# JingwenWang95/DSP-SLAM

Hardware: AMD Instinct MI355X
Metric: objects/sec (2000 pts, 64-D code, 10 GN iters) (higher is better)
Workload: dtype f32 + f16 classifier

## Files before the change

dsp_slam_amd/csrc/mlp_kernel.hip:

```cpp
#include "dsp_internal.h"
#include "mlp_common.h"

namespace dsp {

#define FOR16(M) M(0) M(1) M(2) M(3) M(4) M(5) M(6) M(7) M(8) M(9) M(10) M(11) M(12) M(13) M(14) M(15)

template <int MODE>
__global__ __launch_bounds__(256, 1) void mlp_kernel(const MlpArgs a) {
    constexpr bool BWD = MODE >= 2;
    constexpr bool MASKS = MODE != 0;
    constexpr bool DOFWD = MODE != 3;
    extern __shared__ __attribute__((aligned(16))) char smem[];
    const int tid = threadIdx.x;
    const int lane = tid & 63;
    const int wave = __builtin_amdgcn_readfirstlane(tid >> 6);
    const int g = lane >> 4;
    const int pl = lane & 15;

    const DecoderLds lds = carve_lds(smem);
    float* const bias_l = lds.bias;
    float* const cb_l = lds.cb;
    unsigned short* const mask_l = lds.mask;
    char* ring_ptr = smem + LDS_HEAD_BYTES + (MASKS ? MASK_BYTES : 0);
    const unsigned ring0 = lds_addr(ring_ptr);

    const int n_tiles = *a.n_tiles;
    const int tile0 = a.tile_begin ? *a.tile_begin : 0;
    if (tile0 + (int)blockIdx.x >= n_tiles) return;
    if (a.clk && blockIdx.x == 0 && tid == 0) { a.clk[0] = clock64(); a.clk[1] = wall_clock64(); }
    stage_bias_table(a, bias_l, tid);

    int issue_pos = 0, issue_slot = 0, rd_slot = 0;
    const char* wbase = reinterpret_cast<const char*>(a.wstream) + wave * 4096;
    const unsigned lane_off = lane * 16;
    const int total_chunks = a.total_chunks;
    const char* isrc = wbase;
    unsigned idst = ring0 + wave * 4096;
    auto issue_next = [&]() {
        issue_pos = (issue_pos + 1 == total_chunks) ? 0 : issue_pos + 1;
        issue_slot = (issue_slot + 1 == NBUF) ? 0 : issue_slot + 1;
        isrc = wbase + (size_t)issue_pos * CHUNK_BYTES;
        idst = ring0 + issue_slot * CHUNK_BYTES + wave * 4096;
    };
    auto issue = [&]() {
        glds_quarter(isrc, lane_off, idst);
        issue_next();
    };
#pragma unroll
    for (int i = 0; i < NBUF - 1; ++i) issue();
    asm volatile("s_waitcnt vmcnt(%0)\n\ts_barrier" ::"n"(GLDS_PER_CHUNK * (NBUF - 2)) : "memory");
    f32x4 abuf[2 * PAIR_READS];
    static_assert(PAIR_READS == 2, "the prologue below reads the first group");
    abuf[0] = *reinterpret_cast<const f32x4*>(ring_ptr + lane * 16);
    abuf[1] = *reinterpret_cast<const f32x4*>(ring_ptr + lane * 16 + 1024);

    float sin_[128];
    f32x4 acc[32];
#pragma unroll
    for (int i = 0; i < 128; ++i) sin_[i] = 0.f;
#pragma unroll
    for (int i = 0; i < 32; ++i) acc[i] = (f32x4){0.f, 0.f, 0.f, 0.f};

    for (int tile = tile0 + blockIdx.x; tile < n_tiles; tile += gridDim.x) {
        const int4 td = a.tiles[tile];
        const int local = wave * WAVE_PTS + pl;
        const bool valid = local < td.y;
        const int pidx = td.x + (valid ? local : 0);
        const int src = (MODE <= 1 && a.index) ? a.index[pidx] : pidx;
        float4 pt = a.pts[src];
        float old_lp = 1.0f, guard_tol = 0.f;
        if (MODE <= 1 && a.guard) {
            if (valid && g == 0) old_lp = a.out_sdf[a.index ? src : pidx + td.w];
            guard_tol = 0.5f * __uint_as_float(a.guard[(size_t)td.z * a.guard_stride]);
        }
        if (!valid) pt = make_float4(0.f, 0.f, 0.f, 0.f);
        if (DOFWD) {
            stage_code_bias(a, cb_l, td.z, tid);
            __syncthreads();
#pragma unroll
            for (int o = 0; o < 8; ++o) {
                float pre[16];
#pragma unroll
                for (int j = 0; j < 4; ++j) {
                    const f32x4 p4 = layer0_rows(a, bias_l, cb_l, g, 16 * (4 * o + j), pt);
#pragma unroll
                    for (int r = 0; r < 4; ++r) pre[4 * j + r] = p4[r];
                }
                if (MASKS) {
                    unsigned bits = 0;
#pragma unroll
                    for (int k = 15; k >= 0; --k) push_mask_bit(bits, pre[k]);
                    mask_l[(0 * 8 + o) * 256 + tid] = (unsigned short)bits;
                }
#pragma unroll
                for (int k = 0; k < 16; ++k) sin_[16 * o + k] = relu1(pre[k]);
            }
        }
        float skipc[16];
        float skipx[3];
        float y = 0.f;
        float gfirst = 0.f;
#pragma unroll
        for (int i = 0; i < 16; ++i) skipc[i] = 0.f;
        skipx[0] = skipx[1] = skipx[2] = 0.f;

        auto seed_backward = [&](int slot) {
            const float d = 1.f - y * y;
#pragma unroll
            for (int o = 0; o < 8; ++o) {
                const unsigned bits = mask_l[(slot * 8 + o) * 256 + tid];
#pragma unroll
                for (int j = 0; j < 4; ++j) {
                    const f32x4 s4 = backward_seed_rows(a, bias_l, g, 4 * o + j, bits >> (4 * j), d);
#pragma unroll
                    for (int r = 0; r < 4; ++r) sin_[16 * o + 4 * j + r] = s4[r];
                }
            }
        };
        if (MODE == 3) {
            const int sidx = __float_as_int(pt.w);
            import_masks<8>(mask_words(a, sidx, g), valid, mask_l, tid);
            y = valid ? a.sdf_in[sidx] : 0.f;
            seed_backward(a.seed_slot);
        }

        for (int ps = 0; ps < a.n_pass; ++ps) {
            const PassDesc pd = a.pass[ps];
            if (pd.kind == 2) reinject_xyz(sin_, g, a.lat_tile, pt);
            else if (BWD && pd.kind == 5) gfirst = first_layer_xyz_grad(a, bias_l, g, sin_);

#pragma unroll
            for (int og = 0; og < 8; ++og) {
                if (og < pd.nog) {
                    f32x4 bias4[4];
                    if (pd.bias_row != -1) {
                        const float* bp = pass_bias_vec(pd.bias_row, bias_l, cb_l) + 64 * og + 4 * g;
#pragma unroll
                        for (int j = 0; j < 4; ++j) bias4[j] = *reinterpret_cast<const f32x4*>(bp + 16 * j);
                    } else {
#pragma unroll
                        for (int j = 0; j < 4; ++j) bias4[j] = (f32x4){0.f, 0.f, 0.f, 0.f};
                    }
#pragma unroll
                    for (int c = 0; c < 8; ++c) {
                        if (c < pd.nchunks) {
                            const int nx_slot = (rd_slot + 1 == NBUF) ? 0 : rd_slot + 1;
                            const char* cb = ring_ptr + rd_slot * CHUNK_BYTES + lane * 16;
                            const char* nb = ring_ptr + nx_slot * CHUNK_BYTES + lane * 16;
#pragma unroll
                            for (int s = 0; s < KSTEPS_PER_CHUNK; ++s) {
                                if (s == KSTEPS_PER_CHUNK / 2) {
                                    asm volatile("s_waitcnt vmcnt(%0)\n\ts_barrier" ::"n"(GLDS_PER_CHUNK * (NBUF - 3)) : "memory");
                                }
                                constexpr int RG = PAIR_READS;
                                if ((s % RG) == 0) {
                                    __builtin_amdgcn_s_waitcnt(0xC07F);
                                    __builtin_amdgcn_sched_barrier(0);
#pragma unroll
                                    for (int q = 0; q < RG; ++q) {
                                        const int sp = s + RG + q;
                                        abuf[sp % (2 * RG)] = (sp < KSTEPS_PER_CHUNK)
                                                           ? *reinterpret_cast<const f32x4*>(cb + sp * 1024)
                                                           : *reinterpret_cast<const f32x4*>(nb + (sp - KSTEPS_PER_CHUNK) * 1024);
                                    }
                                }
                                const f32x4 av = abuf[s % (2 * PAIR_READS)];
                                const float b = sin_[16 * c + s];
                                acc[4 * og + 0] = MFMA16(av.x, b, (c == 0 && s == 0) ? bias4[0] : acc[4 * og + 0]);
                                if (s == KSTEPS_PER_CHUNK / 2 + 0) { glds_set_dst(idst); glds_piece_m0<0>(isrc, lane_off, idst); };
                                if (s == KSTEPS_PER_CHUNK / 2 + 1) glds_piece_m0<1>(isrc, lane_off, idst);
                                if (s == KSTEPS_PER_CHUNK / 2 + 2) glds_piece_m0<2>(isrc, lane_off, idst);
                                if (s == KSTEPS_PER_CHUNK / 2 + 3) { glds_piece_m0<3>(isrc, lane_off, idst); issue_next(); }
                                acc[4 * og + 1] = MFMA16(av.y, b, (c == 0 && s == 0) ? bias4[1] : acc[4 * og + 1]);
                                acc[4 * og + 2] = MFMA16(av.z, b, (c == 0 && s == 0) ? bias4[2] : acc[4 * og + 2]);
                                acc[4 * og + 3] = MFMA16(av.w, b, (c == 0 && s == 0) ? bias4[3] : acc[4 * og + 3]);
                                __builtin_amdgcn_sched_barrier(0);
                            }
                            rd_slot = nx_slot;
                        }
                    }
                }
            }

#pragma unroll
            for (int og = 0; og < 8; ++og) {
                if (og < pd.nog) {
                    float v[16];
#pragma unroll
                    for (int j = 0; j < 4; ++j) {
                        v[4 * j + 0] = acc[4 * og + j].x; v[4 * j + 1] = acc[4 * og + j].y;
                        v[4 * j + 2] = acc[4 * og + j].z; v[4 * j + 3] = acc[4 * og + j].w;
                    }
                    if (pd.relu) {
                        if (MASKS) {
                            unsigned bits = 0;
#pragma unroll
                            for (int k = 15; k >= 0; --k) push_mask_bit(bits, v[k]);
                            mask_l[(pd.mask_slot * 8 + og) * 256 + tid] = (unsigned short)bits;
                        }
#pragma unroll
                        for (int k = 0; k < 16; ++k) v[k] = relu1(v[k]);
                    } else if (BWD && pd.mask_slot >= 0) {
                        if (pd.kind == 4) capture_skip_rows(a.lat_tile, og, v, skipx, skipc);
                        const unsigned bits = mask_l[(pd.mask_slot * 8 + og) * 256 + tid];
#pragma unroll
                        for (int k = 0; k < 16; ++k) v[k] = ((bits >> k) & 1u) ? v[k] : 0.f;
                    }
#pragma unroll
                    for (int k = 0; k < 16; ++k) sin_[16 * og + k] = v[k];
                }
            }

            if (DOFWD && ps == a.n_fwd - 1) {
                y = final_layer_sdf(a, bias_l, g, sin_);
                if (!BWD) {
                    if (a.guard) prepass_guard_tol(a, td.z, valid && g == 0, old_lp, y, guard_tol);
                    if (valid && g == 0) a.out_sdf[a.index ? src : pidx + td.w] = y;
                    if (MODE == 1 && valid && y > -a.th && y < a.th) {
                        export_masks<8>(mask_words(a, src, g), mask_l, tid);
                    }
                } else {
                    seed_backward(pd.mask_slot);
                }
            }
        }

        if (BWD) {
            write_jgrad_row(a.out_grad + (size_t)(pidx + td.w) * GRAD_STRIDE, valid, g, pl, sin_, skipc, skipx[0], skipx[1], skipx[2], gfirst, y);
            if (MODE == 2 && a.sdf_scatter && tile >= *a.scatter_tile_begin) scatter_sdf(a, td.z, valid && g == 3, pt, y);
        }
        asm volatile("s_waitcnt vmcnt(0)" ::: "memory");
    }
    asm volatile("s_waitcnt vmcnt(0)" ::: "memory");
    if (a.clk && blockIdx.x == 0 && tid == 0) { a.clk[2] = clock64(); a.clk[3] = wall_clock64(); }
}

static void (*const MLP_KERNELS[4])(const MlpArgs) = {mlp_kernel<0>, mlp_kernel<1>, mlp_kernel<2>, mlp_kernel<3>};

size_t mlp_lds_bytes(int mode) { return LDS_HEAD_BYTES + (mode != 0 ? MASK_BYTES : 0) + NBUF * CHUNK_BYTES; }

hipError_t mlp_prepare_device() {
    for (int i = 0; i < 4; ++i) {
        const hipError_t e = hipFuncSetAttribute(reinterpret_cast<const void*>(MLP_KERNELS[i]), hipFuncAttributeMaxDynamicSharedMemorySize, (int)mlp_lds_bytes(i));
        if (e != hipSuccess) return e;
    }
    return hipSuccess;
}

hipError_t launch_mlp(int mode, const MlpArgs& args, int n_blocks, hipStream_t stream) {
    hipLaunchKernelGGL(MLP_KERNELS[mode], dim3(n_blocks), dim3(256), mlp_lds_bytes(mode), stream, args);
    return hipGetLastError();
}

}
```

Measured before the change: 120.3.

## Double-buffer MFMA accumulators and seed bias tiles inside the MFMA stream

Replaces the 32-register accumulator array with two ping-pong 4-tile accumulator sets plus a separate output array. The bias seeding of the next output group and the copy-out of the previous group are interleaved into the first chunk's MFMA steps. A zero vector in LDS replaces the branch for passes without bias. The aim is to hide the bias loads and the conditional accumulator initialisation behind MFMA latency, at the cost of an extra register copy per tile, extra LDS, and possible register pressure.

After: 121.8, median of 6. 1.3% higher.

```diff
diff --git a/dsp_slam_amd/csrc/mlp_kernel.hip b/dsp_slam_amd/csrc/mlp_kernel.hip
--- a/dsp_slam_amd/csrc/mlp_kernel.hip
+++ b/dsp_slam_amd/csrc/mlp_kernel.hip
@@ -2,6 +2,8 @@
 #include "mlp_common.h"
 
 namespace dsp {
+
+constexpr int ZERO_VEC_BYTES = WIDTH * 4;
 
 #define FOR16(M) M(0) M(1) M(2) M(3) M(4) M(5) M(6) M(7) M(8) M(9) M(10) M(11) M(12) M(13) M(14) M(15)
 
@@ -23,11 +25,13 @@
     unsigned short* const mask_l = lds.mask;
     char* ring_ptr = smem + LDS_HEAD_BYTES + (MASKS ? MASK_BYTES : 0);
     const unsigned ring0 = lds_addr(ring_ptr);
+    float* const zero_l = reinterpret_cast<float*>(ring_ptr + NBUF * CHUNK_BYTES);
 
     const int n_tiles = *a.n_tiles;
     const int tile0 = a.tile_begin ? *a.tile_begin : 0;
     if (tile0 + (int)blockIdx.x >= n_tiles) return;
     if (a.clk && blockIdx.x == 0 && tid == 0) { a.clk[0] = clock64(); a.clk[1] = wall_clock64(); }
+    if (tid < ZERO_VEC_BYTES / 16) reinterpret_cast<float4*>(zero_l)[tid] = make_float4(0.f, 0.f, 0.f, 0.f);
     stage_bias_table(a, bias_l, tid);
 
     int issue_pos = 0, issue_slot = 0, rd_slot = 0;
@@ -55,11 +59,14 @@
     abuf[1] = *reinterpret_cast<const f32x4*>(ring_ptr + lane * 16 + 1024);
 
     float sin_[128];
-    f32x4 acc[32];
+    f32x4 acc[2][4];
+    f32x4 outv[32];
 #pragma unroll
     for (int i = 0; i < 128; ++i) sin_[i] = 0.f;
 #pragma unroll
-    for (int i = 0; i < 32; ++i) acc[i] = (f32x4){0.f, 0.f, 0.f, 0.f};
+    for (int i = 0; i < 32; ++i) outv[i] = (f32x4){0.f, 0.f, 0.f, 0.f};
+#pragma unroll
+    for (int i = 0; i < 8; ++i) acc[i >> 2][i & 3] = (f32x4){0.f, 0.f, 0.f, 0.f};
 
     for (int tile = tile0 + blockIdx.x; tile < n_tiles; tile += gridDim.x) {
         const int4 td = a.tiles[tile];
@@ -129,18 +136,21 @@
             if (pd.kind == 2) reinject_xyz(sin_, g, a.lat_tile, pt);
             else if (BWD && pd.kind == 5) gfirst = first_layer_xyz_grad(a, bias_l, g, sin_);
 
+            auto pin_vgpr = [](f32x4& t) __attribute__((always_inline)) { asm volatile("" : "=v"(t) : "0"(t)); };
+            const float* const seed_src = (pd.bias_row == -1 ? zero_l : pass_bias_vec(pd.bias_row, bias_l, cb_l)) + 4 * g;
+            auto seed_tile = [&](int og, int j) __attribute__((always_inline)) {
+                acc[og & 1][j] = *reinterpret_cast<const f32x4*>(seed_src + 64 * og + 16 * j);
+            };
+            auto read_out = [&](int og, int j) __attribute__((always_inline)) {
+                f32x4 t = acc[og & 1][j];
+                pin_vgpr(t);
+                outv[4 * og + j] = t;
+            };
+#pragma unroll
+            for (int j = 0; j < 4; ++j) seed_tile(0, j);
 #pragma unroll
             for (int og = 0; og < 8; ++og) {
                 if (og < pd.nog) {
-                    f32x4 bias4[4];
-                    if (pd.bias_row != -1) {
-                        const float* bp = pass_bias_vec(pd.bias_row, bias_l, cb_l) + 64 * og + 4 * g;
-#pragma unroll
-                        for (int j = 0; j < 4; ++j) bias4[j] = *reinterpret_cast<const f32x4*>(bp + 16 * j);
-                    } else {
-#pragma unroll
-                        for (int j = 0; j < 4; ++j) bias4[j] = (f32x4){0.f, 0.f, 0.f, 0.f};
-                    }
 #pragma unroll
                     for (int c = 0; c < 8; ++c) {
                         if (c < pd.nchunks) {
@@ -166,14 +176,21 @@
                                 }
                                 const f32x4 av = abuf[s % (2 * PAIR_READS)];
                                 const float b = sin_[16 * c + s];
-                                acc[4 * og + 0] = MFMA16(av.x, b, (c == 0 && s == 0) ? bias4[0] : acc[4 * og + 0]);
+                                f32x4 (&ac)[4] = acc[og & 1];
+                                ac[0] = MFMA16(av.x, b, ac[0]);
                                 if (s == KSTEPS_PER_CHUNK / 2 + 0) { glds_set_dst(idst); glds_piece_m0<0>(isrc, lane_off, idst); };
                                 if (s == KSTEPS_PER_CHUNK / 2 + 1) glds_piece_m0<1>(isrc, lane_off, idst);
                                 if (s == KSTEPS_PER_CHUNK / 2 + 2) glds_piece_m0<2>(isrc, lane_off, idst);
                                 if (s == KSTEPS_PER_CHUNK / 2 + 3) { glds_piece_m0<3>(isrc, lane_off, idst); issue_next(); }
-                                acc[4 * og + 1] = MFMA16(av.y, b, (c == 0 && s == 0) ? bias4[1] : acc[4 * og + 1]);
-                                acc[4 * og + 2] = MFMA16(av.z, b, (c == 0 && s == 0) ? bias4[2] : acc[4 * og + 2]);
-                                acc[4 * og + 3] = MFMA16(av.w, b, (c == 0 && s == 0) ? bias4[3] : acc[4 * og + 3]);
+                                constexpr int SSTEP[4] = {2, 4, 6, 12};
+#pragma unroll
+                                for (int j = 0; j < 4; ++j) {
+                                    if (og > 0 && c == 0 && s == 2 * j + 1) read_out(og - 1, j);
+                                    if (og < 7 && c == 0 && s == SSTEP[j]) seed_tile(og + 1, j);
+                                }
+                                ac[1] = MFMA16(av.y, b, ac[1]);
+                                ac[2] = MFMA16(av.z, b, ac[2]);
+                                ac[3] = MFMA16(av.w, b, ac[3]);
                                 __builtin_amdgcn_sched_barrier(0);
                             }
                             rd_slot = nx_slot;
@@ -185,11 +202,15 @@
 #pragma unroll
             for (int og = 0; og < 8; ++og) {
                 if (og < pd.nog) {
+                    if (og == pd.nog - 1) {
+#pragma unroll
+                        for (int j = 0; j < 4; ++j) read_out(og, j);
+                    }
                     float v[16];
 #pragma unroll
                     for (int j = 0; j < 4; ++j) {
-                        v[4 * j + 0] = acc[4 * og + j].x; v[4 * j + 1] = acc[4 * og + j].y;
-                        v[4 * j + 2] = acc[4 * og + j].z; v[4 * j + 3] = acc[4 * og + j].w;
+                        v[4 * j + 0] = outv[4 * og + j].x; v[4 * j + 1] = outv[4 * og + j].y;
+                        v[4 * j + 2] = outv[4 * og + j].z; v[4 * j + 3] = outv[4 * og + j].w;
                     }
                     if (pd.relu) {
                         if (MASKS) {
@@ -237,7 +258,7 @@
 
 static void (*const MLP_KERNELS[4])(const MlpArgs) = {mlp_kernel<0>, mlp_kernel<1>, mlp_kernel<2>, mlp_kernel<3>};
 
-size_t mlp_lds_bytes(int mode) { return LDS_HEAD_BYTES + (mode != 0 ? MASK_BYTES : 0) + NBUF * CHUNK_BYTES; }
+size_t mlp_lds_bytes(int mode) { return LDS_HEAD_BYTES + (mode != 0 ? MASK_BYTES : 0) + NBUF * CHUNK_BYTES + ZERO_VEC_BYTES; }
 
 hipError_t mlp_prepare_device() {
     for (int i = 0; i < 4; ++i) {
```
